# cvxopt/smcp

Hardware: AMD Instinct MI355X
Metric: Newton KKT solves/sec (higher is better)
Workload: dtype f64; 1 GPU; synth50k nested block-arrow SDP n=50000, 8073 cliques, m=100; kktsolver=chol, n=50000, cliques=8073, m=100, blkval_doubles=2493568, update_doubles=10689536, parallelism=single

## Files before the change

### smcp_amd/csrc/capi.hip

```cpp
#include <hip/hip_runtime.h>
#include <memory>
#include <unordered_map>

#include <algorithm>
#include <chrono>
#include <cstdio>
#include <cstring>
#include <map>
#include <new>
#include <string>
#include <cxxabi.h>
#include <cstdlib>
#include <atomic>
#include <thread>
#include <type_traits>
#include <vector>

#include "../../include/smcp_amd.h"
#include "constraints.hpp"
#include "context.hpp"
#include "hostpar.hpp"
#include "switches.hpp"
#include "front_generic.hip"
#include "front_mfma.hip"
// ... 352 lines not shown
  const auto& lp = c->S.levptr;
  const int64_t l = std::upper_bound(lp.begin(), lp.end(), off) - lp.begin() - 1;
  return (l >= 0 && l < (int64_t)c->lev_namax.size()) ? c->lev_namax[l] : 0;
}

void gather_all(csp_ctx* c, const double* x, int64_t ldx, int nrhs, double* updbase, hipStream_t st) {
  TreeArgs a = tree_args(c);
  for_levels_down(c, [&](const int32_t* lev, int cnt) {
    a.lev = lev;
    launch(c, KID_gather_level, k_gather_level, dim3(cnt, nrhs, gather_parts(namax_of(c, lev), (int64_t)cnt * nrhs, c->D.ncu)), dim3(NT), st, a, x, ldx, updbase);
  });
}

int prepare_yaa(csp_ctx* c, const double* Y, bool need_fac, hipStream_t st, bool need_inv = false, bool allow_partial = false);
void complete_fac(csp_ctx* c, hipStream_t st);


constexpr size_t LDS_LIMIT = 160 * 1024 - 2048;

bool cache_off() {
  static int nocache = -1;
  if (nocache < 0) { const char* e = sw_str("SMCP_NOCACHE"); nocache = (e && e[0] == '1') ? 1 : 0; }
  return nocache == 1;
}

bool use_generic(const csp_ctx* c) {
  static int g = -1;
  if (g < 0) { const char* e = sw_str("SMCP_GENERIC"); g = (e && e[0] == '1') ? 1 : 0; }
  return g == 1 || (c && c->deterministic);
}

MfmaArgs mfma_args(csp_ctx* c, const double* ysc, int ymode, int nrhs) {
  MfmaArgs a;
  a.t = tree_args(c);
  a.t.lev = c->D.lev2idx;
  a.LK = c->D.lk;
  a.ysc = ysc;
  a.ymode = ymode;
  a.nnmax = a.namax = 0;
  a.nchmax = a.panmax = a.pkmax = a.plansum = 0;
  a.nrhs = nrhs;
  { static int sk = -1; if (sk < 0) { const char* e = sw_str("SMCP_SKIP"); sk = e ? atoi(e) : 0; } a.skip = sk; }
  a.dbg = (a.skip & 64) ? (unsigned long long*)(c->D.red + 768) : nullptr;
  a.lfd = c->D.lfd;
  a.dn = 0; a.dld = 0;
  a.kc_ptr = nullptr; a.kc_off = nullptr; a.kc_val = nullptr; a.kc_ids = nullptr;
  a.sp_rt = c->D.sp_rt; a.sp_mk = c->D.sp_mk;
  a.kc_stride = 0; a.kc_j0 = 0;
  a.nnmin = 0;
  a.grp_ptr = nullptr; a.grp_list = nullptr; a.chskip = nullptr; a.famt_ngrp = 0;
  a.fz_on = 0; a.fz_nat = 0; a.fz_cnn = 0; a.fz_stride = 0; a.fz_recl = 0;
  a.fz_tab = nullptr; a.fz_no = nullptr; a.fz_slot = nullptr; a.fz_ptr = nullptr; a.fz_pk = nullptr; a.fz_s = nullptr;
  a.level = 0; a.nS = 0; a.famna = a.fampan = a.fampk = a.famcna = a.famnn = a.famcnn = 0;
  return a;
}

int rhs_groups(int ncl, int nrhs, int target) {
  int g = (target + ncl - 1) / ncl;
  return std::max(1, std::min(g, nrhs));
}

template <class F>
void for_level_classes(csp_ctx* c, int64_t l, MfmaArgs a, F f, int set = 0) {
  const LevelClass& L = set ? c->sets[set].lvl[l] : c->lvl[l];
  const int32_t* base = set ? c->sets[set].lev2 + c->sets[set].off[l] : c->D.lev2idx + c->S.levptr[l];
  if (L.nI) {
    a.t.lev = base;
    a.nnmax = L.nnmaxI;
    a.namax = L.namaxI;
    a.nchmax = L.nchmaxI;
    a.panmax = L.panmaxI;
    a.pkmax = L.pkmaxI;
    a.plansum = L.plansumI;
    a.level = (int)l; a.nS = (int)L.nS; a.famna = L.famna; a.fampan = L.fampan; a.fampk = L.fampk; a.famcna = L.famcna; a.famnn = L.famnn; a.famcnn = L.famcnn;
    size_t lds = (size_t)mfma_lds_doubles(L.nnmaxI, L.namaxI) * sizeof(double);
    f(true, a, (int)L.nI, lds, lds > 48 * 1024 ? 512 : 256);
  }
  if (L.nII) {
    a.t.lev = base + L.nI;
    a.level = (int)l;
    a.nnmax = L.nnmaxII;
    a.nnmin = L.nnminII;
    a.namax = L.namaxII;
    a.nchmax = L.nchmaxII;
    f(false, a, (int)L.nII, (size_t)0, 1024);
  }
}


template <class F>
void for_all_large(csp_ctx* c, MfmaArgs a, F f) {
  if (!c->D.nII_total) return;
  a.t.lev = c->D.lev3idx + c->D.nI_total;
  a.nnmax = c->D.nnmaxII_all;
  a.namax = c->D.namaxII_all;
  f(a, (int)c->D.nII_total);
}

bool use_large() {
  static int g = -1;
  if (g < 0) { const char* e = sw_str("SMCP_LARGE"); g = (e && e[0] == '0') ? 0 : 1; }
  return g == 1;
}
inline unsigned umax1(int x) { return (unsigned)std::max(1, x); }
static int fact_threads(const MfmaArgs& am, int thr, int kind) {
  static int t[3] = {0, 0, 0};
// ... 605 lines not shown
  switch (nat) {
    case 1: ecap = famt_grp_ecap<1>(cnn); break;
    case 2: ecap = famt_grp_ecap<2>(cnn); break;
    case 3: ecap = famt_grp_ecap<3>(cnn); break;
    case 4: ecap = famt_grp_ecap<4>(cnn); break;
  }
  return ecap >= FAMT_GMAX * (FAMT_TCAP / 2);
}
template <int NAT>
bool launch_famt(csp_ctx* c, const MfmaArgs& a, int cnt, int nrhs, double* U, int64_t ldu, hipStream_t st) {
  DeviceCtx& D = c->D;
  if (a.famt_ngrp > 0) {
    const int cnn = std::max(1, a.famcnn);
    const FamtL L = famt_layout<NAT>(8 * cnn);
    const int ecap = famt_grp_ecap<NAT>(cnn);
    static bool attrg = false;
    bool ok = !famt_disabled() && D.lg_request && D.fam_maxterms <= FAMT_TCAP / 2 && ecap >= FAMT_GMAX * (FAMT_TCAP / 2);
    if (ok && !attrg) {
      ok = hipFuncSetAttribute((const void*)k_fam_terms_grp<NAT>, hipFuncAttributeMaxDynamicSharedMemorySize, 160 * 1024 - 1024) == hipSuccess &&
           hipFuncSetAttribute((const void*)k_famt_prep<NAT>, hipFuncAttributeMaxDynamicSharedMemorySize, 160 * 1024 - 1024) == hipSuccess;
      attrg = ok;
    }
    const int64_t need = (int64_t)cnt * (FAMT_HDR + L.total);
    if (ok && dev_grow(&D.famc, &D.famc_len, need, D.mem, st)) ok = false;
    if (!ok) {
      fprintf(stderr, "smcp_amd: grouped family sweep not launchable\n");
      if (!c->launch_err) c->launch_err = -1;
      return true;
    }
    const int gy = std::min(65535, (nrhs + 7) / 8);
    launch_lds(c, KID_famt_prep, k_famt_prep<NAT>, dim3(cnt), dim3(512), (size_t)famt_prep_doubles<NAT>(cnn) * sizeof(double), st, a, D.famc, cnn, (int32_t*)nullptr);
    launch_lds(c, KID_fam_terms_grp, k_fam_terms_grp<NAT>, dim3(a.famt_ngrp, gy), dim3(512), (size_t)(160 * 1024 - 1024), st, a, U, ldu,
               (const double*)D.famc, cnn, (const int32_t*)D.kc_ij, ecap);
    D.lg_nochild = true;
    return true;
  }
  if (famt_disabled() || !D.lg_request) return false;
  const int cnn = std::max(1, a.famcnn);
  const FamtL L = famt_layout<NAT>(8 * cnn);
  const int64_t lim = (160 * 1024 - 1024) / 8;
  const int64_t fixed = L.total + FAMT_NW * famt_desc_doubles() + 6;
  if (!famt_terms_ok(D)) return false;
  if (fixed + 9 * 4 + 64 > lim) return false;
  const int64_t prep_doubles = famt_prep_doubles<NAT>(cnn);
  if (prep_doubles > lim) return false;
  static bool attr = false;
  if (!attr) {
    if (hipFuncSetAttribute((const void*)k_fam_terms<NAT>, hipFuncAttributeMaxDynamicSharedMemorySize, 160 * 1024 - 1024) != hipSuccess) return false;
    if (hipFuncSetAttribute((const void*)k_famt_prep<NAT>, hipFuncAttributeMaxDynamicSharedMemorySize, 160 * 1024 - 1024) != hipSuccess) return false;
    attr = true;
  }
  const int64_t need = (int64_t)cnt * (FAMT_HDR + L.total);
  if (dev_grow(&D.famc, &D.famc_len, need, D.mem, st)) return false;
  const int ncu = D.ncu;
  int g = 1;
  int64_t best = -1;
  for (int gc = 1; gc <= std::min(nrhs, 32); ++gc) {
    const int64_t rounds = ((int64_t)cnt * gc + ncu - 1) / ncu;
    const int64_t passes = (nrhs + gc - 1) / gc;
    const int64_t cost = rounds * (2 * ((passes + FAMT_NW - 1) / FAMT_NW) + 1);
    if (best < 0 || cost < best) { best = cost; g = gc; }
  }
  static int genv = -1;
  if (genv < 0) { const char* e = sw_str("SMCP_FAMT_G"); genv = e ? atoi(e) : 0; }
  if (genv > 0) g = std::min(genv, nrhs);
  const int passes = (nrhs + g - 1) / g;
  const double avg = 9.0 * (double)D.cnnz / ((double)c->S.nsn * (double)std::max<int64_t>(1, D.m));
  int tabpasses = std::min(passes, 113);
  auto tail = [&](int tp) { return (int64_t)2 * ((tp * 9 + 1) & ~1) / 2 + 2; };
  while (tabpasses > 4 && fixed + tail(tabpasses) + (int64_t)(1.5 * 1.5 * avg * tabpasses) + 8 > lim) tabpasses = (tabpasses + 1) / 2;
  const int64_t left = lim - fixed - tail(tabpasses) - 4;
  const int ecap = (int)std::max<int64_t>(0, (left * 2) / 3 - 2);
  if (9 * D.kc_maxlist > ecap) return false;
  if (a.fz_on) {
    static bool attrz = false;
    if (!attrz) attrz = hipFuncSetAttribute((const void*)k_fam_terms<NAT, false>, hipFuncAttributeMaxDynamicSharedMemorySize, 160 * 1024 - 1024) == hipSuccess;
    if (attrz && D.fz_slot) {
      launch_lds(c, KID_famt_prep, k_famt_prep<NAT>, dim3(cnt), dim3(512), (size_t)prep_doubles * sizeof(double), st, a, D.famc, cnn, D.fz_slot);
      launch_lds(c, KID_fam_terms, k_fam_terms<NAT, false>, dim3(cnt, g), dim3(64 * FAMT_NW), (size_t)lim * 8, st, a, U, ldu,
                 (const double*)D.famc, cnn, (const int32_t*)D.kc_ij, tabpasses, ecap);
      D.lg_nochild = true;
      c->fz_live = true; c->fz_nat = NAT; c->fz_cnn = cnn; c->fz_recl = (int64_t)(FAMT_HDR + L.total);
      return true;
    }
  }
  launch_lds(c, KID_famt_prep, k_famt_prep<NAT>, dim3(cnt), dim3(512), (size_t)prep_doubles * sizeof(double), st, a, D.famc, cnn, (int32_t*)nullptr);
  launch_lds(c, KID_fam_terms, k_fam_terms<NAT>, dim3(cnt, g), dim3(64 * FAMT_NW), (size_t)lim * 8, st, a, U, ldu,
             (const double*)D.famc, cnn, (const int32_t*)D.kc_ij, tabpasses, ecap);
  D.lg_nochild = true;
  return true;
}
inline bool fam2_disabled() {
  static int off = -1;
  if (off < 0) { const char* e = sw_str("SMCP_FAM2"); off = (e && e[0] == '0') ? 1 : 0; }
  return off != 0;
}
bool try_fam2(csp_ctx* c, const MfmaArgs& a, int cnt, int nrhs, double* U, int64_t ldu, hipStream_t st) {
  if (fam2_disabled() || !a.kc_ptr || !c->D.kc_ij || a.ymode != 2 || !a.ysc) return false;
  if (c->D.cnnz > (int64_t)4 * c->S.nsn * std::max<int64_t>(1, c->D.m)) return false;
  const int nat = std::max(1, (a.famna + 15) / 16);
  const bool k2 = a.famnn <= 8;
  switch (nat) {
    case 1: if (launch_famt<1>(c, a, cnt, nrhs, U, ldu, st)) return true; break;
    case 2: if (launch_famt<2>(c, a, cnt, nrhs, U, ldu, st)) return true; break;
    case 3: if (launch_famt<3>(c, a, cnt, nrhs, U, ldu, st)) return true; break;
    case 4: if (launch_famt<4>(c, a, cnt, nrhs, U, ldu, st)) return true; break;
  }
  switch (nat) {
    case 1: return k2 ? launch_fam2<1, 2>(c, a, cnt, nrhs, U, ldu, st) : launch_fam2<1, 4>(c, a, cnt, nrhs, U, ldu, st);
    case 2: return k2 ? launch_fam2<2, 2>(c, a, cnt, nrhs, U, ldu, st) : launch_fam2<2, 4>(c, a, cnt, nrhs, U, ldu, st);
    case 3: return k2 ? launch_fam2<3, 2>(c, a, cnt, nrhs, U, ldu, st) : launch_fam2<3, 4>(c, a, cnt, nrhs, U, ldu, st);
    case 4: return k2 ? launch_fam2<4, 2>(c, a, cnt, nrhs, U, ldu, st) : launch_fam2<4, 4>(c, a, cnt, nrhs, U, ldu, st);
  }
  return false;
}
bool try_fam(csp_ctx* c, const MfmaArgs& a, int cnt, int nrhs, double* U, int64_t ldu, hipStream_t st) {
  if (try_fam2(c, a, cnt, nrhs, U, ldu, st)) return true;
  if (a.famt_ngrp > 0) {
    fprintf(stderr, "smcp_amd: grouped family sweep refused by try_fam2 (conditions of hess_up_fast and try_fam2 disagree)\n");
    if (!c->launch_err) c->launch_err = -1;
    return true;
  }
  if (a.ysc == c->D.fac) complete_fac(c, st);
  return a.kc_ptr ? try_fam_sp<true>(c, a, cnt, nrhs, U, ldu, st) : try_fam_sp<false>(c, a, cnt, nrhs, U, ldu, st);
}

bool try_lfsp(csp_ctx* c, const MfmaArgs& a, int cnt, int nrhs, double* U, int64_t ldu, hipStream_t st, const csp_ctx::LfspGroups* grp = nullptr) {
  static int on = -1;
  if (on < 0) { const char* e = sw_str("SMCP_LFSP"); on = (e && e[0] == '0') ? 0 : 1; }
  DeviceCtx& D = c->D;
  if (!on || !a.kc_ptr || a.nchmax != 0 || a.ymode != 2 || !a.ysc || a.nnmax > 64 || a.namax > 128) return false;
  if (D.kc_maxlist_large <= 0 || D.kc_maxlist_large > LFSP_ECAP || !D.lfsp_cnt) return false;
  const bool exact = D.lfsp_exact;
  if (!D.sp_rt) {
    if (dev_alloc(&D.sp_rt, std::max<int64_t>(c->S.updlen(), 1), D.mem)) return false;
    if (dev_alloc(&D.sp_mk, std::max<int64_t>(c->S.blklen(), 1), D.mem)) return false;
  }
  MfmaArgs b = a;
  b.sp_rt = D.sp_rt; b.sp_mk = D.sp_mk;
  if (D.sp_fac_gen != D.fac_gen || D.sp_lk_gen != D.lk_gen) {
// ... 1480 lines not shown
```

### smcp_amd/csrc/front_famt.hip

```cpp
#include <hip/hip_runtime.h>

namespace smcp {

struct FamtL { int oLi, onK, onMK, oRt, oZero, oCN, oCA, oCM, total; };
template <int NAT>
__host__ __device__ inline FamtL famt_layout(int ncol) {
  constexpr int NA = 16 * NAT;
  FamtL L{};
  int o = 0;
  L.oLi = o; o += 256;
  L.onK = o; o += NA * 16;
  L.onMK = o; o += NA * 16;
  L.oRt = o; o += NA * NA;
  L.oZero = o; o += NA;
  L.oCN = o; o += ncol * 16;
  L.oCA = o; o += ncol * NA;
  L.oCM = o; o += ncol * NA;
  L.total = o;
  return L;
}
typedef unsigned int famt_u2 __attribute__((ext_vector_type(2)));
__device__ inline __amdgpu_buffer_rsrc_t famt_rsrc(double* base, int doubles) {
  return __builtin_amdgcn_make_buffer_rsrc(base, 0, doubles * 8, 0x00020000);
}
#ifndef SMCP_FAMT_AUX
#define SMCP_FAMT_AUX 0
#endif
__device__ inline void famt_store(__amdgpu_buffer_rsrc_t r, bool ok, int pos, double v) {
  __builtin_amdgcn_raw_buffer_store_b64(__builtin_bit_cast(famt_u2, v), r, ok ? pos * 8 : -1, 0, SMCP_FAMT_AUX);
}
#ifndef SMCP_FAMT_NW
#define SMCP_FAMT_NW 12
#endif
constexpr int FAMT_NW = SMCP_FAMT_NW;
constexpr int FAMT_HDR = 32;
constexpr int FAMT_TCAP = 96;
constexpr int FAMT_TMAX = 384;
constexpr int FAMT_CHILD = 128;
constexpr int FAMT_UNIT = 1 << 30;
#ifndef SMCP_FAMT_UB
#define SMCP_FAMT_UB 8
#endif
constexpr int FAMT_UB = SMCP_FAMT_UB;

template <int NAT>
__host__ __device__ inline int famt_prep_doubles(int cnn) { constexpr int NA = 16 * NAT; return NA * NA + NA * 16 + 256 + 8 * (NA + 16 + cnn * NA); }

template <int NAT>
__global__ void __launch_bounds__(512) k_famt_prep(MfmaArgs a, double* famt, int cnn, int32_t* fz_slot) {
  extern __shared__ __attribute__((aligned(16))) double smem[];
  constexpr int NA = 16 * NAT;
  const int ncol = 8 * cnn;
  const FamtL L = famt_layout<NAT>(ncol);
  const int k = a.t.lev[blockIdx.x];
  const CliqueDesc d = a.t.cl[k];
  const int nn = d.nn, na = d.na, nf = nn + na, nch = d.chend - d.chbeg;
  const int tid = threadIdx.x, lane = tid & 63, wave = tid >> 6;
  double* const sRt = smem;
  double* const snK = sRt + NA * NA;
  double* const sLi = snK + NA * 16;
  double* const qt = sLi + 256 + wave * (NA + 16 + cnn * NA);
  double* const sCA = qt + NA + 16;
  double* const out = famt + (int64_t)blockIdx.x * (FAMT_HDR + L.total);
  double* const T = out + FAMT_HDR;
  const int myck = lane < nch ? a.t.chidx[d.chbeg + lane] : 0;
  const int mynn = lane < nch ? a.t.cl[myck].nn : 0;
  int inc = mynn;
#pragma unroll
  for (int o = 1; o < 8; o <<= 1) { const int v = __shfl_up(inc, o); if (lane >= o) inc += v; }
  const int colbase = __shfl(inc - mynn, min(wave, 7));
  const int ck = __shfl(myck, min(wave, 7));
  for (int e = tid; e < NA * NA + NA * 16 + 256; e += 512) smem[e] = 0.0;
  __syncthreads();
  {
    const double* lk = a.LK + d.blk;
    const double* ys = a.ysc + d.upd;
    for (int e = tid; e < nf * nn; e += 512) {
      const int i = e % nf, j = e / nf;
      if (i >= nn) snK[(i - nn) + j * NA] = -lk[e];
      else if (i >= j) sLi[i + j * 16] = lk[e];
    }
    batched_loop<8>(tid, na * na, 512, [=](int e) { return ys[e]; },
                    [=](int e, double v) {
                      const int i = e % na, p = e / na;
                      if (i >= p) sRt[p + i * NA] = v;
                    });
  }
  __syncthreads();
  for (int e = tid; e < 256; e += 512) T[L.oLi + e] = sLi[e];
  for (int e = tid; e < NA * 16; e += 512) T[L.onK + e] = snK[e];
  for (int e = tid; e < NA * NA; e += 512) T[L.oRt + e] = sRt[e];
  for (int e = tid; e < NA; e += 512) T[L.oZero + e] = 0.0;
// ... 41 lines not shown
            const double rt = sRt[p + q * NA];
#pragma unroll
            for (int x = 0; x < 8; ++x) s8[x] += rt * sCA[min(j0 + x, cnn - 1) * NA + q];
          }
#pragma unroll
        for (int x = 0; x < 8; ++x) if (j0 + x < nnc) T[L.oCM + (colbase + j0 + x) * NA + p] = s8[x];
      }
    if (lane == 0) {
      int* const hdr = reinterpret_cast<int*>(out) + 16 + 6 * wave;
      hdr[0] = ck; hdr[1] = nnc; hdr[2] = nac; hdr[3] = colbase; hdr[4] = 0; hdr[5] = 0;
    }
  } else if (wave < 8 && lane == 0) {
    int* const hdr = reinterpret_cast<int*>(out) + 16 + 6 * wave;
    hdr[0] = -1; hdr[1] = 1; hdr[2] = 0; hdr[3] = 0; hdr[4] = 0; hdr[5] = 0;
  }
  {
    const int used = __shfl(inc, 7);
    for (int e = tid; e < (ncol - used) * 16; e += 512) T[L.oCN + used * 16 + e] = 0.0;
    for (int e = tid; e < (ncol - used) * NA; e += 512) { T[L.oCA + used * NA + e] = 0.0; T[L.oCM + used * NA + e] = 0.0; }
  }
  if (tid == 0) {
    if (fz_slot && a.fz_no && a.fz_no[k] >= 0) fz_slot[a.fz_no[k]] = (int32_t)blockIdx.x;
    int* const hdr = reinterpret_cast<int*>(out);
    hdr[0] = k; hdr[1] = nn; hdr[2] = na; hdr[3] = nch;
    hdr[4] = (int)(d.blk & 0xffffffffll); hdr[5] = (int)(d.blk >> 32);
    hdr[6] = 0; hdr[7] = 0;
    hdr[8] = (int)(d.updp & 0xffffffffll); hdr[9] = (int)(d.updp >> 32);
  }
}

template <int NTH>
__device__ inline void famt_copy_tables(double* smem, const double* src, int total, int tid) {
  const double2* const s2 = reinterpret_cast<const double2*>(src);
  double2* const d2 = reinterpret_cast<double2*>(smem);
  const int n2 = total >> 1;
  for (int e0 = tid; e0 < n2; e0 += NTH * 8) {
    double2 v[8];
#pragma unroll
    for (int x = 0; x < 8; ++x) v[x] = s2[min(e0 + x * NTH, n2 - 1)];
#pragma unroll
    for (int x = 0; x < 8; ++x) if (e0 + x * NTH < n2) d2[e0 + x * NTH] = v[x];
  }
}

__host__ __device__ inline int famt_desc_doubles() { return FAMT_TCAP * 3; }

template <int NAT, bool UPD = true>
__global__ void __launch_bounds__(64 * FAMT_NW) k_fam_terms(MfmaArgs a, double* u, int64_t ldu, const double* famt, int cnn,
                                                   const int32_t* kc_ij, int tabpasses, int ecap) {
  extern __shared__ __attribute__((aligned(16))) double smem[];
  constexpr int NA = 16 * NAT, NW = FAMT_NW, NTH = 64 * NW;
  const int ncol = 8 * cnn;
  const FamtL L = famt_layout<NAT>(ncol);
  const double* const fc = famt + (int64_t)blockIdx.x * (FAMT_HDR + L.total);
  const int32_t* const hdr = reinterpret_cast<const int32_t*>(fc);
  const int k = hdr[0], nn = hdr[1], na = hdr[2], nch = hdr[3], nf = nn + na;
  const int64_t pblk = (int64_t)(uint32_t)hdr[4] | ((int64_t)hdr[5] << 32);
  const int64_t pupdp = (int64_t)(uint32_t)hdr[8] | ((int64_t)hdr[9] << 32);
  const int tid = threadIdx.x;
  const int lane = tid & 63, l15 = lane & 15, kq = lane >> 4;
  const int wave = __builtin_amdgcn_readfirstlane(tid >> 6);
  const int nmem = nch + 1;
  const int gy = (int)gridDim.y;
  const int npass = ((int)a.nrhs - (int)blockIdx.y + gy - 1) / gy;
  double* const dS = smem + L.total + wave * famt_desc_doubles();
  int* const dI = reinterpret_cast<int*>(dS + FAMT_TCAP);
  int* const misc = reinterpret_cast<int*>(smem + L.total + NW * famt_desc_doubles());
  int* const epfit = misc;
  int* const cdim = misc + 2;
  int* const tab = misc + 12;
  double* const lval = reinterpret_cast<double*>(tab + 2 * ((tabpasses * nmem + 1) & ~1));
  int* const lpk = reinterpret_cast<int*>(lval + ecap);

  famt_copy_tables<NTH>(smem, fc + FAMT_HDR, L.total, tid);
  if (tid < 8) cdim[tid] = tid < nch ? (hdr[16 + 6 * tid + 1] | (hdr[16 + 6 * tid + 3] << 8)) : 1;

  for (int q0 = 0; q0 < npass;) {
    const int epmax = min(tabpasses, npass - q0), npairs = epmax * nmem;
    __syncthreads();
    if (tid == 0) *epfit = epmax;
    int myp0[2] = {0, 0};
#pragma unroll
    for (int h = 0; h < 2; ++h) {
      const int idx = tid + NTH * h;
      if (idx < npairs) {
        const int qq = idx / nmem, mem = idx - qq * nmem;
        const int r = (int)blockIdx.y + (q0 + qq) * gy;
        const int j = a.kc_ids ? a.kc_ids[a.kc_j0 + r] : a.kc_j0 + r;
        const int ck = mem ? hdr[16 + 6 * (mem - 1)] : k;
        const int32_t* kp = a.kc_ptr + (int64_t)ck * a.kc_stride;
        myp0[h] = kp[j];
        tab[2 * idx] = kp[j + 1] - myp0[h];
      }
    }
    __syncthreads();
    if (wave == 0) {
      const int per = (npairs + 63) / 64, b = lane * per;
      int sum = 0;
      for (int x = 0; x < per; ++x) sum += (b + x < npairs) ? tab[2 * (b + x)] : 0;
      int incl = sum;
#pragma unroll
      for (int o = 1; o < 64; o <<= 1) { const int v = __shfl_up(incl, o); if (lane >= o) incl += v; }
      int run = incl - sum;
      for (int x = 0; x < per; ++x)
        if (b + x < npairs) {
          const int c = tab[2 * (b + x)];
          tab[2 * (b + x) + 1] = run;
          run += c;
          if (run > ecap) atomicMin(epfit, (b + x) / nmem);
        }
    }
    __syncthreads();
    const int ep = max(1, *epfit);
#pragma unroll
    for (int h = 0; h < 2; ++h) {
      const int idx = tid + NTH * h;
      if (idx < ep * nmem) {
        const int c = tab[2 * idx], p0 = myp0[h], off = tab[2 * idx + 1];
        const int qq = idx / nmem, mem = idx - qq * nmem;
        (void)qq;
        const int mnn = mem ? hdr[16 + 6 * (mem - 1) + 1] : 0;
        const int mck = mem ? hdr[16 + 6 * (mem - 1)] : 0;
        const int32_t* const mrel = a.t.relidx + a.t.cl[mem ? mck : k].rel;
        for (int t = 0; t < c && off + t < ecap; ++t) {
          const int ij = kc_ij[p0 + t];
          const int i = ij & 0xffff, jc = ij >> 16;
          int pk = i | (jc << 8);
          if (mem && i >= mnn) pk |= mrel[i - mnn] << 16;
          lpk[off + t] = pk;
          lval[off + t] = a.kc_val[p0 + t];
        }
      }
    }
    __builtin_amdgcn_s_waitcnt(0x0F70);
    __syncthreads();

    for (int qq = wave; qq < ep; qq += NW) {
      const int r = (int)blockIdx.y + (q0 + qq) * gy;
      const int* const trow = tab + 2 * qq * nmem;
      int cntm = lane < nmem ? trow[2 * lane] : 0;
      int incl = cntm;
#pragma unroll
      for (int o = 1; o < 16; o <<= 1) { const int v = __shfl_up(incl, o); if (lane >= o) incl += v; }
      const int Ttot = min(__builtin_amdgcn_readlane(incl, 15), FAMT_TMAX);
      const int ndp = max(1, (Ttot + FAMT_TCAP / 2 - 1) / (FAMT_TCAP / 2));
      auto build = [&](int dp) {
        const int e = dp * (FAMT_TCAP / 2) + lane;
        const int T = min(FAMT_TCAP / 2, Ttot - dp * (FAMT_TCAP / 2));
        int mem = 0, base = 0;
#pragma unroll
        for (int mm = 0; mm < 8; ++mm) {
          const int up = __builtin_amdgcn_readlane(incl, mm);
          if (e >= up) { mem = mm + 1; base = up; }
        }
        if (lane < T) {
          const int where = trow[2 * mem + 1];
          const int pk = lpk[where + (e - base)];
          const double v = lval[where + (e - base)];
          const int i = pk & 0xff, jc = (pk >> 8) & 0xff, rl = (pk >> 16) & 0xff;
          int vx, vy;
          double s;
          if (mem == 0) { vx = i; vy = jc; s = i == jc ? 0.5 * v : v; }
          else {
            const int cd = cdim[mem - 1], nnc = cd & 0xff, cb = cd >> 8;
            if (i >= nnc) { vx = FAMT_CHILD + cb + jc; vy = rl; s = -v; }
            else { vx = FAMT_CHILD + cb + i; vy = FAMT_CHILD + cb + jc; s = i == jc ? 0.5 * v : v; }
          }
          auto img = [&](int vid, int& on, int& oa, int& om, int& ui) {
            if (vid >= FAMT_CHILD) { const int g = vid - FAMT_CHILD; on = L.oCN + 16 * g; oa = L.oCA + NA * g; om = L.oCM + NA * g; ui = 255; }
            else if (vid < nn) { on = L.oLi + 16 * vid; oa = L.onK + NA * vid; om = L.onMK + NA * vid; ui = 255; }
            else { on = L.oZero; oa = L.oZero; om = L.oRt + NA * (vid - nn); ui = vid - nn; }
          };
          int nx, ax, mx, ux, ny, ay, my, uy;
          img(vx, nx, ax, mx, ux);
          img(vy, ny, ay, my, uy);
          dS[2 * lane] = s; dS[2 * lane + 1] = s;
          int4 w0 = {nx | (ax << 16), mx | (ux << 16), ny | (ay << 16), uy};
          int4 w1 = {ny | (ay << 16), my | (uy << 16), nx | (ax << 16), ux};
          reinterpret_cast<int4*>(dI)[2 * lane] = w0;
          reinterpret_cast<int4*>(dI)[2 * lane + 1] = w1;
        }
        if (lane < 4 && 2 * T + lane < ((2 * T + 3) & ~3)) {
          dS[2 * T + lane] = 0.0;
          int4 z = {L.oZero | (L.oZero << 16), L.oZero | (255 << 16), L.oZero | (L.oZero << 16), 255};
          reinterpret_cast<int4*>(dI)[2 * T + lane] = z;
        }
        __builtin_amdgcn_fence(__ATOMIC_RELEASE, "wavefront"); __builtin_amdgcn_wave_barrier(); __builtin_amdgcn_fence(__ATOMIC_ACQUIRE, "wavefront");
      };
      build(0);
      const __amdgpu_buffer_rsrc_t rP = famt_rsrc(u + (int64_t)r * ldu + pblk, nf * nn);
      const __amdgpu_buffer_rsrc_t rU = famt_rsrc(a.t.updp + (int64_t)r * a.t.updplen + pupdp, (na * (na + 1)) >> 1);
// ... 517 lines not shown
```

### smcp_amd/csrc/front_mfma.hip

```cpp
#include <hip/hip_runtime.h>

namespace smcp {

typedef double d4 __attribute__((ext_vector_type(4)));

template <class FA, class FB, class FC>
__device__ inline void wg_mma(int M, int N, int Kd, FA A, FB B, FC store, bool lower_only = false, int rot = 0) {
  const int lane = threadIdx.x & 63, nw = blockDim.x >> 6;
  const int wave = ((threadIdx.x >> 6) + nw - (rot % nw)) % nw;
  const int mt = (M + 15) >> 4, nt = (N + 15) >> 4;
  const int l15 = lane & 15, kq = lane >> 4;
  for (int t = wave; t < mt * nt; t += nw) {
    const int tm = t % mt, tn = t / mt;
    if (lower_only && tm < tn) continue;
    const int m = tm * 16 + l15, nb = tn * 16 + l15;
    d4 acc = {0.0, 0.0, 0.0, 0.0};
    constexpr int KU = 2;
    for (int k0 = 0; k0 < Kd; k0 += 4 * KU) {
      double av[KU], bv[KU];
#pragma unroll
      for (int u = 0; u < KU; ++u) {
        const int k = k0 + 4 * u + kq;
        const bool kin = k < Kd;
        av[u] = (kin && m < M) ? A(m, k) : 0.0;
        bv[u] = (kin && nb < N) ? B(k, nb) : 0.0;
      }
#pragma unroll
      for (int u = 0; u < KU; ++u)
        if (k0 + 4 * u < Kd) acc = __builtin_amdgcn_mfma_f64_16x16x4f64(bv[u], av[u], acc, 0, 0, 0);
    }
#pragma unroll
    for (int r = 0; r < 4; ++r) {
      const int n = tn * 16 + kq + 4 * r;
      if (m < M && n < N) store(m, n, acc[r]);
    }
  }
}

template <int UNR, class LoadF, class UseF>
__device__ inline void batched_loop(int begin, int end, int step, LoadF load, UseF use) {
  for (int e0 = begin; e0 < end; e0 += step * UNR) {
    decltype(load(0)) v[UNR];
#pragma unroll
    for (int u = 0; u < UNR; ++u) {
      const int e = e0 + u * step;
      if (e < end) v[u] = load(e);
    }
#pragma unroll
    for (int u = 0; u < UNR; ++u) {
      const int e = e0 + u * step;
      if (e < end) use(e, v[u]);
    }
  }
}

struct MfmaArgs {
  TreeArgs t;
  const double* LK;
  const double* ysc;
  int ymode;
  int nnmax, namax;
  int nrhs;
  int nchmax, panmax, pkmax, plansum;
  int skip;
  unsigned long long* dbg;
  double* lfd;
  int dn; int64_t dld;
  const int32_t* kc_ptr; const int32_t* kc_off; const double* kc_val; const int32_t* kc_ids;
  int kc_stride, kc_j0;
  const double* sp_rt; const double* sp_mk;
  int level, nS, famna, fampan, fampk, famcna, famnn, famcnn;
  int nnmin;
  const int32_t* grp_ptr; const int32_t* grp_list; const uint8_t* chskip;
  int famt_ngrp;
  int fz_on, fz_nat, fz_cnn, fz_stride;
  int64_t fz_recl;
  const double* fz_tab; const int32_t* fz_no; const int32_t* fz_slot; const int32_t* fz_ptr; const int32_t* fz_pk; const double* fz_s;
};

__device__ __host__ inline int padld(int x) { return x | 1; }

__host__ __device__ inline int64_t mfma_lds_doubles(int nn, int na) {
  int64_t lk = padld(na), ll = padld(nn), lf = padld(nn + na);
  int64_t nnc = nn;
  return lk * nnc + ll * nnc + lk * (int64_t)na + lf * nnc + ll * nnc + lk * nnc + lk * nnc + ll * nnc + lk * (int64_t)na + 16 * 16 + 8 + (na + 2) / 2;
}

enum : int { WK_K = 1, WK_LI = 2, WK_Y = 4, WK_F = 8, WK_FNN = 16, WK_E = 32, WK_G = 64, WK_T = 128, WK_U = 256, WK_ALL = 511 };
constexpr int WK_CHOL = WK_F | WK_U;
constexpr int WK_PINV = WK_K | WK_LI | WK_E | WK_U;
constexpr int WK_DOWN0 = WK_ALL & ~(WK_Y | WK_FNN);
constexpr int WK_COMPL = WK_Y | WK_F | WK_FNN | WK_E | WK_G | WK_T;
__host__ __device__ inline int64_t mfma_lds_doubles_for(int mask, int nn, int na) {
  const int64_t lk = padld(na), ll = padld(nn), lf = padld(nn + na), nnc = nn;
  int64_t t = 0;
  if (mask & WK_K) t += lk * nnc;
  if (mask & WK_LI) t += ll * nnc;
  if (mask & WK_Y) t += lk * (int64_t)na;
  if (mask & WK_F) t += lf * nnc;
  if (mask & WK_FNN) t += ll * nnc;
  if (mask & WK_E) t += lk * nnc;
  if (mask & WK_G) t += lk * nnc;
  if (mask & WK_T) t += ll * nnc;
  if (mask & WK_U) t += lk * (int64_t)na;
  return t + 16 * 16 + 8 + (na + 2) / 2;
}
__host__ __device__ inline int64_t completion_lds_doubles(int nn, int na) {
  return mfma_lds_doubles_for(WK_COMPL, nn, na) + (nn > 16 ? 16 * 128 : 0);
}

struct Work {
  const double* K; int ldk;
  const double* Li; int ldl;
  const double* Y; int ldy;
  double* F; int ldf;
  double* Fnn; int ldn;
  double* E; int lde;
  double* G; int ldg;
  double* T; int ldt;
  double* U; int ldu;
  double* D16;
};

template <bool LDS, int MASK = WK_ALL>
__device__ inline Work make_work(const MfmaArgs& a, const CliqueDesc& d, double* smem, int k, int r) {
  Work w;
  const int nn = d.nn, na = d.na, nf = nn + na;
  if (LDS) {
    const int lk = padld(a.namax), ll = padld(a.nnmax), lf = padld(a.nnmax + a.namax);
    double* p = smem;
// ... 1259 lines not shown
```

### smcp_amd/csrc/switches.hpp

```cpp
#pragma once
#include <cstdio>
#include <cstdlib>
#include <cstring>
#include <string>

extern char** environ;

namespace smcp {

struct Switch { const char* name; const char* dflt; const char* doc; };

static const Switch SWITCHES[] = {
  {"SMCP_GENERIC", "0", "1: any-size fixed-order kernels of front_generic.hip for every tree operation (as CSP_TUNE_DETERMINISTIC)"},
  {"SMCP_LARGE", "1", "0: no tiled large-front kernels (fronts beyond LDS take the one-workgroup HBM kernels)"},
  {"SMCP_NOCACHE", "0", "1: nothing derived from (L, Y) is reused between calls"},
  {"SMCP_FORK", "1", "0: no side streams, everything on the caller's stream"},
  {"SMCP_AUX_PRIO", "1", "0: side stream 0 (few-workgroup chains) at default instead of highest priority"},
  {"SMCP_AUX_PRIO1", "1", "0: side stream 1 (filler work) at default instead of lowest priority"},
  {"SMCP_EVENT_SYSFENCE", "0", "1: internal events with the default system-scope release (12 us per hand-over instead of 7)"},
  {"SMCP_SCALING_OVERLAP", "1", "0: csp_cholesky_projected_inverse as its three steps one after the other"},
  {"SMCP_CHOL_PREP", "1", "0: k_prep_lk in a launch of its own instead of inside k_chol_mfma (narrow supernodes)"},
  {"SMCP_FAC_PARTIAL", "1", "0: chol(Y_AA) of the family children always formed by the fused scaling point"},
  {"SMCP_MID", "1", "0: per-step kernels instead of k_mid_chol / k_lf_diag_inv for fronts of at most 272 rows"},
  {"SMCP_TOP_FUSED", "1", "0: k_mid_chol, and k_lf_diag_inv / k_lf_trtri for the inverse at the scaling point, instead of the register-resident k_top_chol for fronts of at most 208 rows"},
// ... 1 lines not shown
  {"SMCP_N16", "1", "0: no shape-specialised k_hess_up_n16"},
  {"SMCP_OLDLDS", "0", "1: k_hess_up_mfma<true> instead of the padded / n16 kernels"},
  {"SMCP_DOWN_W", "1", "0: k_hess_down_mfma instead of the one-wave k_hess_down_w"},
  {"SMCP_DOWN_FAM", "1", "most right-hand sides of a root -> leaves sweep that take the one-launch family kernel k_hess_down_fam (0: never; the per-level k_hess_down_w launches)"},
  {"SMCP_UP_FAM", "1", "most dense right-hand sides of a leaves -> root sweep that take the resident family kernel k_hess_up_fam1, the level-0 cliques outside the families riding along (0: never; k_hess_up_fam and a launch of their own for those cliques)"},
  {"SMCP_SCALING_FAM", "1", "0: per-level k_chol_mfma / k_pinv_mfma launches for the families of the scaling point instead of one k_chol_fam / k_pinv_fam launch each way"},
  {"SMCP_FAM", "1", "0: no family kernels (per-level sweeps with the update exchange through HBM)"},
  {"SMCP_FAM2", "1", "0: no sparse-input family kernels (k_fam_sparse, k_fam_terms): k_hess_up_fam"},
  {"SMCP_FAMT", "1", "0: no entry-driven family sweep k_fam_terms (k_fam_sparse instead)"},
  {"SMCP_FZ", "1", "0: the family parents' packed updates go through HBM (k_fam_terms writes, the extend-add reads) instead of being formed by k_lf_assemble_fz"},
  {"SMCP_FAMT_GROUP", "1", "0: no sibling groups of family parents (k_fam_terms_grp)"},
  {"SMCP_LFSP", "1", "0: dense phases instead of the sparse-input sweep k_lfsp_up of childless large fronts"},
  {"SMCP_LFSP_GROUP", "1", "0: no sibling groups in k_lfsp_up"},
  {"SMCP_ZSP", "1", "0: dense first phase of wide childless fronts instead of k_lf_zsp"},
  {"SMCP_LEAFGRAM", "1", "0: never the closed-form Gram blocks of the family children (k_leaf_tables / k_leaf_pairs)"},
  {"SMCP_LG_SIDE", "1", "0: leaf Gram blocks after the sweep on the caller's stream instead of beside the top phases"},
  {"SMCP_GRAM_EARLY", "0", "1: the Gram chunks of the levels 0 / 1 rows on the side branch beside the top fronts' phase kernels (measured slower: 3.37 against 3.22 ms per step)"},
  {"SMCP_LG_EARLY", "1", "0: leaf Gram blocks beside the phase kernels of the top fronts instead of from the start of the sweep"},
  {"SMCP_FACI_LDS", "1", "0: inverse Y_AA factors of the small fronts by block rows against HBM (k_factor_inverse) instead of in LDS"},
  {"SMCP_FZ_TAIL", "1", "0: every (front, right-hand side) pair of the fused extend-add is one workgroup's task, also in a thin last round"},
  {"SMCP_GRAM", "1", "0: reference (two-sweep) formulation of the Schur complement instead of the Gram formulation"},
  {"SMCP_SCM", "1", "0: column-sparse constraints swept like the others (no SCMcolumn2 route)"},
  {"SMCP_TRSM_MM", "1", "0: csp_trsm through the generic level kernels instead of tile products"},
  {"SMCP_TRMM_MM", "1", "0: no MFMA tile products in csp_trmm (every front on the FMA kernels); 2: tile products for the large fronts only, also from 32 columns on"},
  {"SMCP_SYR2K_MM", "1", "0: no MFMA tile products in csp_syr2k (every front on the FMA kernel); 2: tile products for the large fronts only, whatever the rank (read on every call)"},
  {"SMCP_SYMM_MM", "1", "0: no MFMA tile products in csp_symm (every front on the FMA kernel); 2: tile products for the large fronts only, whatever the column count (read on every call)"},
  {"SMCP_LOWRANK_MM", "1", "0: no MFMA tiles in the Gram products of the low-rank factor (k_lr_gram on the FMA route whatever the shape)"},
  {"SMCP_POTRS_MANY_MM", "1", "0: no MFMA tile products in the block steps of dense_potrs_many / kkt_solve_many (FMA updates whatever the column count; read on every call)"},
  {"SMCP_ALDS", "1", "0: extend-add of large fronts by gather plan only (no LDS streaming kernel)"},
  {"SMCP_ALDS_DYN", "1", "0: one workgroup per (front, right-hand side) instead of the task-drawing grid"},
  {"SMCP_ALDS_FILL", "1", "0: k_panel_fill builds the input panels instead of the extend-add (sgn 3)"},
  {"SMCP_ASM", "plan", "t: tiled extend-add kernel instead of the gather plan"},
  {"SMCP_ROOT_FUSED", "0", "1: fused two-product sweep of fronts without separator (Y_NN explicit: condition squared; studies only)"},
  {"SMCP_PD", "0", "1: four-wave tile products everywhere (no sixteen-wave shape for small launches)"},
  {"SMCP_FLOW", "1", "0: no one-launch blocked Cholesky with in-launch tile dataflow (front_flow.hip): per-step kernels for dense matrices / single fronts beyond 272 rows"},
  {"SMCP_FLOW_WG", "112", "workgroups of that launch (at most 112: four launches fit the chip side by side)"},
  {"SMCP_POTRF_DEFER", "1", "0: kkt_schur_factor factors H at once even under deferred status"},
  {"SMCP_QR_TRSM", "mfma", "f: vector-FMA substitution kernel of kkt_qr instead of the MFMA one"},
  {"SMCP_FTHR_CHOL", "128", "threads of k_chol_mfma on the leaf class"},
  {"SMCP_FTHR_PINV", "256", "threads of k_pinv_mfma on the leaf class"},
  {"SMCP_FTHR_YAA", "64", "threads of k_factor_yaa_lds on the leaf class"},
  {"SMCP_FTHR_YAA_MID", "256", "threads of k_factor_yaa_lds on separator blocks of 33 .. 64 rows"},
  {"SMCP_N16_THR_LEAF", "128", "threads of k_hess_up_n16 for one or two right-hand sides on childless fronts"},
  {"SMCP_DIAG_THREADS", "512", "threads of k_lf_diag"},
  {"SMCP_POTRF_THREADS", "1024", "threads of k_dense_potrf_small"},
  {"SMCP_FZ_THREADS", "1024", "threads of k_lf_assemble_fz (512: eight waves, no register spills, slower)"},
  {"SMCP_PD_WGS", "1", "largest launch, in workgroups per CU, that takes the sixteen-wave tile shape"},
  {"SMCP_ALDS_Z", "0", "workgroups per (front, right-hand side) of the LDS extend-add (0: automatic)"},
  {"SMCP_RHS_SPLIT", "16", "fewest right-hand sides for the two-stream split of a large-front sweep (plain extend-add launch only)"},
  {"SMCP_RHS_PARTS", "2", "parts of that split (2 or 3)"},
  {"SMCP_RHS_SPLIT_DYN", "0", "1: the split also with the task-drawing extend-add"},
  {"SMCP_FAM_MINRHS", "1", "fewest dense right-hand sides for the family kernel"},
  {"SMCP_FAMT_G", "0", "right-hand-side slices per family of k_fam_terms (0: cost model)"},
  {"SMCP_FAM2_STAG", "0", "stagger of k_fam_sparse's groups (studies)"},
  {"SMCP_FAMT_MEAN", "36", "entry-driven family sweeps (k_fam_terms, fused extend-add) up to this many entries per (family, constraint) list ON AVERAGE (lists up to 384 entries, in chunks); beyond: the dense family sweep"},
  {"SMCP_LFSP_OCC", "2", "waves per SIMD the grouped update phase of k_lfsp_up is compiled for (1: 512 registers, no spills; 2: 256, ~100 spilled)"},
  {"SMCP_LFSP_G", "1", "right-hand sides per workgroup of k_lfsp_up"},
  {"SMCP_GRAM_NW", "16", "waves per workgroup of k_gram_diag128 (4, 8 or 16)"},
  {"SMCP_GRAM_MINCHUNK", "512", "fewest stack rows per workgroup of the Gram accumulation"},
  {"SMCP_UPDP_PAD", "0", "doubles of padding between the packed exchange buffers of consecutive right-hand sides"},
  {"SMCP_QR_PASSES", "0", "Cholesky-QR passes of kkt_qr (0: decided by the deviation test)"},
  {"SMCP_QR_P", "1", "positions per lane of the FMA substitution kernel (1 or 2)"},
  {"SMCP_FLOW_STAMPS", "0", "1: per-workgroup time accounts of the one-launch blocked Cholesky on stderr (waits for every launch)"},
  {"SMCP_POISON", "0", "1: every fp64 device buffer of the library (and the exchange buffers of smcp_amd/kkt.py) starts as 4.5e150 (hunting reads of never-written workspace)"},
  {"SMCP_RACE", "0", "seed > 0: delay injection on every internal stream hand-over and one launch in eight (race hunting; results must not change)"},
  {"SMCP_TRACE", "0", "1: every launch named on stderr, by its kernel id and [by the kernel function launched], and waited for (a device fault points at its kernel)"},
  {"SMCP_TIMING", "0", "1: wall-clock marks of the set-up phases on stderr"},
  {"SMCP_OCC", "0", "1: occupancy decisions of k_hess_up_n16 on stderr"},
  {"SMCP_DEBUG_ADDR", "0", "1: addresses of the large allocations on stderr"},
  {"SMCP_CONTIG", "0", "1: large buffers from physically contiguous memory (placement studies: slower)"},
  {"SMCP_SKIP", "0", "phase mask of the sweep kernels (ablation timing; results are wrong)"},
  {"SMCP_GSKIP", "0", "ablation mask of the Gram kernel (results are wrong)"},
  {"SMCP_LGSKIP", "0", "ablation mask of k_leaf_pairs (results are wrong)"},
  {"SMCP_QR_FAKE", "0", "1: timing experiment of the FMA substitution kernel (results are wrong)"},
};

inline void sw_check_environment() {
  static const bool done = [] {
    for (char** e = environ; e && *e; ++e) {
      if (std::strncmp(*e, "SMCP_", 5) != 0) continue;
      const char* eq = std::strchr(*e, '=');
      const std::string name(*e, eq ? (size_t)(eq - *e) : std::strlen(*e));
      if (name.rfind("SMCP_BENCH_", 0) == 0 || name.rfind("SMCP_FUZZ_", 0) == 0 || name == "SMCP_CXXFLAGS" || name == "SMCP_STAMPS" ||
          name == "SMCP_SHARD_KEEP" || name == "SMCP_SHARD_TOP" || name == "SMCP_GIT_SHA" || name == "SMCP_FS_MODE") continue;
      bool known = false;
      for (const Switch& s : SWITCHES) if (name == s.name) known = true;
      if (!known) std::fprintf(stderr, "smcp_amd: unknown switch %s in the environment (see smcp_amd/csrc/switches.hpp)\n", name.c_str());
    }
    return true;
  }();
  (void)done;
}
inline const char* sw_str(const char* name) {
  sw_check_environment();
  bool known = false;
  for (const Switch& s : SWITCHES) if (!std::strcmp(name, s.name)) { known = true; break; }
  if (!known) std::fprintf(stderr, "smcp_amd: switch %s is read but not listed in switches.hpp\n", name);
  return std::getenv(name);
}
inline int sw_on(const char* name, int dflt) { const char* v = sw_str(name); return v ? (v[0] == '0' ? 0 : (v[0] == '1' ? 1 : dflt)) : dflt; }
inline int sw_int(const char* name, int dflt) { const char* v = sw_str(name); return v ? std::atoi(v) : dflt; }

}
```

Baseline: 374.2 KKT solves/s.

## Split last-round families across RHS slices and draw passes dynamically in k_fam_terms

The grid-shape cost model now counts resident workgroups from an occupancy query instead of CU count. When one slice per family is chosen, the families in the last partial round are split across several right-hand-side slices so the tail fills the chip. Inside k_fam_terms, waves now take passes through an LDS atomic counter instead of a fixed stride, which balances uneven per-pass work. The cost is extra index arithmetic, an atomic per pass, and repeated per-family setup work for each split slice.

```diff
diff --git a/smcp_amd/csrc/capi.hip b/smcp_amd/csrc/capi.hip
--- a/smcp_amd/csrc/capi.hip
+++ b/smcp_amd/csrc/capi.hip
@@ -428,6 +428,7 @@
   a.fz_on = 0; a.fz_nat = 0; a.fz_cnn = 0; a.fz_stride = 0; a.fz_recl = 0;
   a.fz_tab = nullptr; a.fz_no = nullptr; a.fz_slot = nullptr; a.fz_ptr = nullptr; a.fz_pk = nullptr; a.fz_s = nullptr;
   a.level = 0; a.nS = 0; a.famna = a.fampan = a.fampk = a.famcna = a.famnn = a.famcnn = 0;
+  a.famt_nfull = 0; a.famt_ns = 0;
   return a;
 }
 
@@ -1139,18 +1140,43 @@
   }
   const int64_t need = (int64_t)cnt * (FAMT_HDR + L.total);
   if (dev_grow(&D.famc, &D.famc_len, need, D.mem, st)) return false;
-  const int ncu = D.ncu;
+  static bool attrz = false;
+  if (a.fz_on && !attrz) attrz = hipFuncSetAttribute((const void*)k_fam_terms<NAT, false>, hipFuncAttributeMaxDynamicSharedMemorySize, 160 * 1024 - 1024) == hipSuccess;
+  const bool fz = a.fz_on && attrz && D.fz_slot;
+  static int occ[2] = {0, 0};
+  if (!occ[fz]) {
+    int nb = 0;
+    const hipError_t e = fz ? hipOccupancyMaxActiveBlocksPerMultiprocessor(&nb, k_fam_terms<NAT, false>, 64 * FAMT_NW, (size_t)lim * 8)
+                            : hipOccupancyMaxActiveBlocksPerMultiprocessor(&nb, k_fam_terms<NAT, true>, 64 * FAMT_NW, (size_t)lim * 8);
+    occ[fz] = (e == hipSuccess && nb > 0) ? nb : 1;
+  }
+  static int senv = -1;
+  if (senv < 0) senv = std::max(0, sw_int("SMCP_FAMT_SLOTS", 0));
+  const int slots = senv > 0 ? senv : std::max(1, D.ncu) * occ[fz];
+  auto wg_cost = [](int64_t p) { return 2 * ((p + FAMT_NW - 1) / FAMT_NW) + 1; };
+  auto last_round_slices = [&](int rem) { return (rem > 0 && cnt > slots) ? std::max(1, std::min(slots / rem, nrhs / FAMT_NW)) : 1; };
   int g = 1;
   int64_t best = -1;
   for (int gc = 1; gc <= std::min(nrhs, 32); ++gc) {
-    const int64_t rounds = ((int64_t)cnt * gc + ncu - 1) / ncu;
-    const int64_t passes = (nrhs + gc - 1) / gc;
-    const int64_t cost = rounds * (2 * ((passes + FAMT_NW - 1) / FAMT_NW) + 1);
+    int64_t cost;
+    if (gc == 1) {
+      const int rem = cnt % slots, s = last_round_slices(rem);
+      cost = (int64_t)(cnt / slots) * wg_cost(nrhs) + (rem ? wg_cost((nrhs + s - 1) / s) : 0);
+    } else {
+      cost = (((int64_t)cnt * gc + slots - 1) / slots) * wg_cost((nrhs + gc - 1) / gc);
+    }
     if (best < 0 || cost < best) { best = cost; g = gc; }
   }
   static int genv = -1;
   if (genv < 0) { const char* e = sw_str("SMCP_FAMT_G"); genv = e ? atoi(e) : 0; }
   if (genv > 0) g = std::min(genv, nrhs);
+  MfmaArgs as = a;
+  as.famt_nfull = cnt; as.famt_ns = 1;
+  int gridx = cnt;
+  if (g == 1 && cnt > slots) {
+    const int rem = cnt % slots, s = last_round_slices(rem);
+    if (s > 1) { as.famt_nfull = cnt - rem; as.famt_ns = s; gridx = as.famt_nfull + rem * s; }
+  }
   const int passes = (nrhs + g - 1) / g;
   const double avg = 9.0 * (double)D.cnnz / ((double)c->S.nsn * (double)std::max<int64_t>(1, D.m));
   int tabpasses = std::min(passes, 113);
@@ -1159,20 +1185,16 @@
   const int64_t left = lim - fixed - tail(tabpasses) - 4;
   const int ecap = (int)std::max<int64_t>(0, (left * 2) / 3 - 2);
   if (9 * D.kc_maxlist > ecap) return false;
-  if (a.fz_on) {
-    static bool attrz = false;
-    if (!attrz) attrz = hipFuncSetAttribute((const void*)k_fam_terms<NAT, false>, hipFuncAttributeMaxDynamicSharedMemorySize, 160 * 1024 - 1024) == hipSuccess;
-    if (attrz && D.fz_slot) {
-      launch_lds(c, KID_famt_prep, k_famt_prep<NAT>, dim3(cnt), dim3(512), (size_t)prep_doubles * sizeof(double), st, a, D.famc, cnn, D.fz_slot);
-      launch_lds(c, KID_fam_terms, k_fam_terms<NAT, false>, dim3(cnt, g), dim3(64 * FAMT_NW), (size_t)lim * 8, st, a, U, ldu,
-                 (const double*)D.famc, cnn, (const int32_t*)D.kc_ij, tabpasses, ecap);
-      D.lg_nochild = true;
-      c->fz_live = true; c->fz_nat = NAT; c->fz_cnn = cnn; c->fz_recl = (int64_t)(FAMT_HDR + L.total);
-      return true;
-    }
+  if (fz) {
+    launch_lds(c, KID_famt_prep, k_famt_prep<NAT>, dim3(cnt), dim3(512), (size_t)prep_doubles * sizeof(double), st, a, D.famc, cnn, D.fz_slot);
+    launch_lds(c, KID_fam_terms, k_fam_terms<NAT, false>, dim3(gridx, g), dim3(64 * FAMT_NW), (size_t)lim * 8, st, as, U, ldu,
+               (const double*)D.famc, cnn, (const int32_t*)D.kc_ij, tabpasses, ecap);
+    D.lg_nochild = true;
+    c->fz_live = true; c->fz_nat = NAT; c->fz_cnn = cnn; c->fz_recl = (int64_t)(FAMT_HDR + L.total);
+    return true;
   }
   launch_lds(c, KID_famt_prep, k_famt_prep<NAT>, dim3(cnt), dim3(512), (size_t)prep_doubles * sizeof(double), st, a, D.famc, cnn, (int32_t*)nullptr);
-  launch_lds(c, KID_fam_terms, k_fam_terms<NAT>, dim3(cnt, g), dim3(64 * FAMT_NW), (size_t)lim * 8, st, a, U, ldu,
+  launch_lds(c, KID_fam_terms, k_fam_terms<NAT>, dim3(gridx, g), dim3(64 * FAMT_NW), (size_t)lim * 8, st, as, U, ldu,
              (const double*)D.famc, cnn, (const int32_t*)D.kc_ij, tabpasses, ecap);
   D.lg_nochild = true;
   return true;
diff --git a/smcp_amd/csrc/front_famt.hip b/smcp_amd/csrc/front_famt.hip
--- a/smcp_amd/csrc/front_famt.hip
+++ b/smcp_amd/csrc/front_famt.hip
@@ -38,6 +38,9 @@
 constexpr int FAMT_TMAX = 384;
 constexpr int FAMT_CHILD = 128;
 constexpr int FAMT_UNIT = 1 << 30;
+#ifndef SMCP_FAMT_DRAW
+#define SMCP_FAMT_DRAW 1
+#endif
 #ifndef SMCP_FAMT_UB
 #define SMCP_FAMT_UB 8
 #endif
@@ -185,7 +188,11 @@
   constexpr int NA = 16 * NAT, NW = FAMT_NW, NTH = 64 * NW;
   const int ncol = 8 * cnn;
   const FamtL L = famt_layout<NAT>(ncol);
-  const double* const fc = famt + (int64_t)blockIdx.x * (FAMT_HDR + L.total);
+  const int bx = (int)blockIdx.x;
+  const bool cut = a.famt_ns > 1 && bx >= a.famt_nfull;
+  const int fam = cut ? a.famt_nfull + (bx - a.famt_nfull) / a.famt_ns : bx;
+  const int sl = cut ? (bx - a.famt_nfull) % a.famt_ns : (int)blockIdx.y;
+  const double* const fc = famt + (int64_t)fam * (FAMT_HDR + L.total);
   const int32_t* const hdr = reinterpret_cast<const int32_t*>(fc);
   const int k = hdr[0], nn = hdr[1], na = hdr[2], nch = hdr[3], nf = nn + na;
   const int64_t pblk = (int64_t)(uint32_t)hdr[4] | ((int64_t)hdr[5] << 32);
@@ -194,12 +201,13 @@
   const int lane = tid & 63, l15 = lane & 15, kq = lane >> 4;
   const int wave = __builtin_amdgcn_readfirstlane(tid >> 6);
   const int nmem = nch + 1;
-  const int gy = (int)gridDim.y;
-  const int npass = ((int)a.nrhs - (int)blockIdx.y + gy - 1) / gy;
+  const int gy = cut ? a.famt_ns : (int)gridDim.y;
+  const int npass = ((int)a.nrhs - sl + gy - 1) / gy;
   double* const dS = smem + L.total + wave * famt_desc_doubles();
   int* const dI = reinterpret_cast<int*>(dS + FAMT_TCAP);
   int* const misc = reinterpret_cast<int*>(smem + L.total + NW * famt_desc_doubles());
   int* const epfit = misc;
+  int* const draw = misc + 1;
   int* const cdim = misc + 2;
   int* const tab = misc + 12;
   double* const lval = reinterpret_cast<double*>(tab + 2 * ((tabpasses * nmem + 1) & ~1));
@@ -211,14 +219,14 @@
   for (int q0 = 0; q0 < npass;) {
     const int epmax = min(tabpasses, npass - q0), npairs = epmax * nmem;
     __syncthreads();
-    if (tid == 0) *epfit = epmax;
+    if (tid == 0) { *epfit = epmax; *draw = 0; }
     int myp0[2] = {0, 0};
 #pragma unroll
     for (int h = 0; h < 2; ++h) {
       const int idx = tid + NTH * h;
       if (idx < npairs) {
         const int qq = idx / nmem, mem = idx - qq * nmem;
-        const int r = (int)blockIdx.y + (q0 + qq) * gy;
+        const int r = sl + (q0 + qq) * gy;
         const int j = a.kc_ids ? a.kc_ids[a.kc_j0 + r] : a.kc_j0 + r;
         const int ck = mem ? hdr[16 + 6 * (mem - 1)] : k;
         const int32_t* kp = a.kc_ptr + (int64_t)ck * a.kc_stride;
@@ -268,8 +276,16 @@
     __builtin_amdgcn_s_waitcnt(0x0F70);
     __syncthreads();
 
+#if SMCP_FAMT_DRAW
+    for (;;) {
+      int qd = 0;
+      if (lane == 0) qd = atomicAdd(draw, 1);
+      const int qq = __builtin_amdgcn_readfirstlane(qd);
+      if (qq >= ep) break;
+#else
     for (int qq = wave; qq < ep; qq += NW) {
-      const int r = (int)blockIdx.y + (q0 + qq) * gy;
+#endif
+      const int r = sl + (q0 + qq) * gy;
       const int* const trow = tab + 2 * qq * nmem;
       int cntm = lane < nmem ? trow[2 * lane] : 0;
       int incl = cntm;
diff --git a/smcp_amd/csrc/front_mfma.hip b/smcp_amd/csrc/front_mfma.hip
--- a/smcp_amd/csrc/front_mfma.hip
+++ b/smcp_amd/csrc/front_mfma.hip
@@ -76,6 +76,7 @@
   int fz_on, fz_nat, fz_cnn, fz_stride;
   int64_t fz_recl;
   const double* fz_tab; const int32_t* fz_no; const int32_t* fz_slot; const int32_t* fz_ptr; const int32_t* fz_pk; const double* fz_s;
+  int famt_nfull, famt_ns;
 };
 
 __device__ __host__ inline int padld(int x) { return x | 1; }
diff --git a/smcp_amd/csrc/switches.hpp b/smcp_amd/csrc/switches.hpp
--- a/smcp_amd/csrc/switches.hpp
+++ b/smcp_amd/csrc/switches.hpp
@@ -77,6 +77,7 @@
   {"SMCP_RHS_SPLIT_DYN", "0", "1: the split also with the task-drawing extend-add"},
   {"SMCP_FAM_MINRHS", "1", "fewest dense right-hand sides for the family kernel"},
   {"SMCP_FAMT_G", "0", "right-hand-side slices per family of k_fam_terms (0: cost model)"},
+  {"SMCP_FAMT_SLOTS", "0", "workgroups of k_fam_terms the chip is taken to hold at a time, for the split of the last round (0: CUs x resident workgroups, from the occupancy query; a value above the family count: no split)"},
   {"SMCP_FAM2_STAG", "0", "stagger of k_fam_sparse's groups (studies)"},
   {"SMCP_FAMT_MEAN", "36", "entry-driven family sweeps (k_fam_terms, fused extend-add) up to this many entries per (family, constraint) list ON AVERAGE (lists up to 384 entries, in chunks); beyond: the dense family sweep"},
   {"SMCP_LFSP_OCC", "2", "waves per SIMD the grouped update phase of k_lfsp_up is compiled for (1: 512 registers, no spills; 2: 256, ~100 spilled)"},
```

Result: no change. 374.3 KKT solves/s, median of 2 (+0.0%).
